# zju3dv/SMAP

Hardware: NVIDIA H100
Metric: end-to-end FPS @832x512 (backbone+association+lift) (higher is better)
Workload: dtype bf16x3 (split-bf16 operands, fp32 accumulate; fp32-faithful)

## Files before the change

### smap_b200/csrc/common.cuh

```cuda
#pragma once
#include <cuda_runtime.h>
#include <cuda_bf16.h>
#include <stdint.h>

#ifndef __CUDA_ARCH_FEAT_SM90_ALL
#if defined(__CUDA_ARCH__)
#error "smap_b200 kernels must be compiled with -gencode arch=compute_90a,code=sm_90a"
#endif
#endif

namespace smapb {

__device__ __forceinline__ uint32_t smem_u32(const void* p) {
    return (uint32_t)__cvta_generic_to_shared(p);
}

__device__ __forceinline__ void mbar_init(uint64_t* bar, uint32_t count) {
    asm volatile("mbarrier.init.shared::cta.b64 [%0], %1;" ::"r"(smem_u32(bar)), "r"(count) : "memory");
}
__device__ __forceinline__ void fence_mbar_init() {
    asm volatile("fence.mbarrier_init.release.cluster;" ::: "memory");
}
__device__ __forceinline__ void fence_proxy_async() {
    asm volatile("fence.proxy.async.shared::cta;" ::: "memory");
}
__device__ __forceinline__ void mbar_arrive_expect_tx(uint64_t* bar, uint32_t bytes) {
    asm volatile("mbarrier.arrive.expect_tx.shared::cta.b64 _, [%0], %1;" ::"r"(smem_u32(bar)), "r"(bytes)
                 : "memory");
}
__device__ __forceinline__ void mbar_arrive(uint64_t* bar) {
    asm volatile("mbarrier.arrive.shared::cta.b64 _, [%0];" ::"r"(smem_u32(bar)) : "memory");
}
__device__ __forceinline__ uint32_t mbar_try_wait(uint64_t* bar, uint32_t parity) {
    uint32_t ok;
    asm volatile(
        "{\n\t.reg .pred p;\n\t"
        "mbarrier.try_wait.parity.shared::cta.b64 p, [%1], %2;\n\t"
        "selp.u32 %0, 1, 0, p;\n\t}"
        : "=r"(ok)
        : "r"(smem_u32(bar)), "r"(parity)
        : "memory");
    return ok;
}
__device__ __forceinline__ void mbar_wait(uint64_t* bar, uint32_t parity) {
    if (mbar_try_wait(bar, parity)) return;
    const long long t0 = clock64();
    while (!mbar_try_wait(bar, parity)) {
        if (clock64() - t0 > 4000000000LL) {
            __trap();
        }
    }
}

__device__ __forceinline__ void bulk_g2s(void* dst_smem, const void* src_gmem, uint32_t bytes, uint64_t* bar) {
    asm volatile(
        "cp.async.bulk.shared::cluster.global.mbarrier::complete_tx::bytes [%0], [%1], %2, [%3];" ::"r"(
            smem_u32(dst_smem)),
        "l"(src_gmem), "r"(bytes), "r"(smem_u32(bar))
        : "memory");
}

__device__ __forceinline__ uint32_t lane_id() { return threadIdx.x & 31; }

__device__ __forceinline__ void pdl_wait() { asm volatile("griddepcontrol.wait;" ::: "memory"); }
__device__ __forceinline__ void pdl_trigger() { asm volatile("griddepcontrol.launch_dependents;" ::: "memory"); }

__device__ __forceinline__ void split_bf16(float v, __nv_bfloat16& hi, __nv_bfloat16& lo) {
    hi = __float2bfloat16_rn(v);
    lo = __float2bfloat16_rn(v - __bfloat162float(hi));
}
__device__ __forceinline__ uint32_t pack_bf16x2(__nv_bfloat16 a, __nv_bfloat16 b) {
    return (uint32_t)__bfloat16_as_ushort(a) | ((uint32_t)__bfloat16_as_ushort(b) << 16);
}
__device__ __forceinline__ float bf16lo_to_f(uint32_t packed) { return __uint_as_float(packed << 16); }
__device__ __forceinline__ float bf16hi_to_f(uint32_t packed) { return __uint_as_float(packed & 0xffff0000u); }

}
```

### smap_b200/csrc/conv_tc.cuh

```cuda
#pragma once
#include <cuda.h>
#include "common.cuh"

namespace smapb {

struct alignas(64) ConvParams {
    CUtensorMap tmA;
    CUtensorMap tmA2;
    CUtensorMap tmB;
    CUtensorMap tmO;
    CUtensorMap tmR[3];
    int Hout, Wout, Nimg;
    int tw_log2, th;
    int tiles_x, tiles_y;
    int Cout;
    int kh, kw, stride, pad_y, pad_x;
    int kchunks;
    int kchunks2, stride2;
    int n_tiles;
    int total_tiles;
    const float* bias;
    int has_res;
    int n_post;
    __nv_bfloat16* out;
    float* out_f32;
    long long plane_stride;
    int relu;
    int reverse;
    int up_mode, up_Hi, up_Wi, up_pw, up_ph;
    long long* dbg;
    long long* dbg_tl;
};

__device__ __forceinline__ void tma_load_5d(uint32_t dst, const CUtensorMap* map, uint64_t* bar, int c0, int c1,
                                            int c2, int c3, int c4) {
    asm volatile(
        "cp.async.bulk.tensor.5d.shared::cluster.global.tile.mbarrier::complete_tx::bytes [%0], [%1, {%3, %4, %5, %6, "
        "%7}], [%2];" ::"r"(dst),
        "l"(map), "r"(smem_u32(bar)), "r"(c0), "r"(c1), "r"(c2), "r"(c3), "r"(c4)
        : "memory");
}
__device__ __forceinline__ void tma_load_4d(uint32_t dst, const CUtensorMap* map, uint64_t* bar, int c0, int c1,
                                            int c2, int c3) {
    asm volatile(
        "cp.async.bulk.tensor.4d.shared::cluster.global.tile.mbarrier::complete_tx::bytes [%0], [%1, {%3, %4, %5, "
        "%6}], [%2];" ::"r"(dst),
        "l"(map), "r"(smem_u32(bar)), "r"(c0), "r"(c1), "r"(c2), "r"(c3)
        : "memory");
}
__device__ __forceinline__ void tma_prefetch_desc(const CUtensorMap* map) {
    asm volatile("prefetch.tensormap [%0];" ::"l"(map) : "memory");
}
__device__ __forceinline__ void tma_store_5d(const CUtensorMap* map, uint32_t src, int c0, int c1, int c2, int c3,
                                             int c4) {
    asm volatile("cp.async.bulk.tensor.5d.global.shared::cta.tile.bulk_group [%0, {%2, %3, %4, %5, %6}], [%1];" ::"l"(map),
                 "r"(src), "r"(c0), "r"(c1), "r"(c2), "r"(c3), "r"(c4)
                 : "memory");
}
__device__ __forceinline__ void bulk_commit() { asm volatile("cp.async.bulk.commit_group;" ::: "memory"); }
template <int N>
__device__ __forceinline__ void bulk_wait_read() {
    asm volatile("cp.async.bulk.wait_group.read %0;" ::"n"(N) : "memory");
}
__device__ __forceinline__ void bulk_wait_all() { asm volatile("cp.async.bulk.wait_group 0;" ::: "memory"); }
__device__ __forceinline__ void epi_bar_sync() { asm volatile("bar.sync 1, 256;" ::: "memory"); }
__device__ __forceinline__ uint32_t lds_u32(uint32_t addr) {
    uint32_t r;
    asm volatile("ld.shared.u32 %0, [%1];" : "=r"(r) : "r"(addr));
    return r;
}
__device__ __forceinline__ void sts_u32(uint32_t addr, uint32_t v) {
    asm volatile("st.shared.u32 [%0], %1;" ::"r"(addr), "r"(v) : "memory");
}
__device__ __forceinline__ uint32_t sw64_off(int r, int j) { return (uint32_t)(r * 64 + ((j ^ ((r >> 1) & 3)) << 4)); }

__device__ __forceinline__ float up_scale(int in, int out) { return out > 1 ? (float)(in - 1) / (float)(out - 1) : 0.f; }
__device__ __forceinline__ int up_src_index(int dst, int in, int out) { return (int)(up_scale(in, out) * (float)dst); }

__device__ __forceinline__ uint32_t cvt_bf16x2(float a, float b) {
    uint32_t w;
    asm("cvt.rn.bf16x2.f32 %0, %1, %2;" : "=r"(w) : "f"(b), "f"(a));
    return w;
}
__device__ __forceinline__ float2 planes_to_f2(uint32_t h, uint32_t l) {
    return make_float2(bf16lo_to_f(h) + bf16lo_to_f(l), bf16hi_to_f(h) + bf16hi_to_f(l));
}

__device__ __forceinline__ uint64_t wgmma_desc_sw128(uint32_t smem_addr) {
    uint64_t d = 0;
    d |= (uint64_t)((smem_addr >> 4) & 0x3FFF);
    d |= (uint64_t)1 << 16;
    d |= (uint64_t)(1024 >> 4) << 32;
    d |= (uint64_t)1 << 62;
    return d;
}
__device__ __forceinline__ void wgmma_fence() { asm volatile("wgmma.fence.sync.aligned;" ::: "memory"); }
__device__ __forceinline__ void wgmma_commit() { asm volatile("wgmma.commit_group.sync.aligned;" ::: "memory"); }
template <int N>
__device__ __forceinline__ void wgmma_wait() {
    asm volatile("wgmma.wait_group.sync.aligned %0;" ::"n"(N) : "memory");
}
__device__ __forceinline__ void wgmma_m64n128(float (&d)[64], uint64_t adesc, uint64_t bdesc, uint32_t accumulate) {
    asm volatile(
        "{\n\t.reg .pred p;\n\tsetp.ne.b32 p, %66, 0;\n\t"
        "wgmma.mma_async.sync.aligned.m64n128k16.f32.bf16.bf16 {%0, %1, %2, %3, %4, %5, %6, %7, %8, %9, %10, %11, %12, "
        "%13, %14, %15, %16, %17, %18, %19, %20, %21, %22, %23, %24, %25, %26, %27, %28, %29, %30, %31, %32, %33, %34, %35, "
        "%36, %37, %38, %39, %40, %41, %42, %43, %44, %45, %46, %47, %48, %49, %50, %51, %52, %53, %54, %55, %56, %57, %58, "
        "%59, %60, %61, %62, %63}, %64, %65, p, 1, 1, 0, 0;\n\t}"
        : "+f"(d[0]), "+f"(d[1]), "+f"(d[2]), "+f"(d[3]), "+f"(d[4]), "+f"(d[5]), "+f"(d[6]), "+f"(d[7]), "+f"(d[8]),
          "+f"(d[9]), "+f"(d[10]), "+f"(d[11]), "+f"(d[12]), "+f"(d[13]), "+f"(d[14]), "+f"(d[15]), "+f"(d[16]),
          "+f"(d[17]), "+f"(d[18]), "+f"(d[19]), "+f"(d[20]), "+f"(d[21]), "+f"(d[22]), "+f"(d[23]), "+f"(d[24]),
          "+f"(d[25]), "+f"(d[26]), "+f"(d[27]), "+f"(d[28]), "+f"(d[29]), "+f"(d[30]), "+f"(d[31]), "+f"(d[32]),
          "+f"(d[33]), "+f"(d[34]), "+f"(d[35]), "+f"(d[36]), "+f"(d[37]), "+f"(d[38]), "+f"(d[39]), "+f"(d[40]),
          "+f"(d[41]), "+f"(d[42]), "+f"(d[43]), "+f"(d[44]), "+f"(d[45]), "+f"(d[46]), "+f"(d[47]), "+f"(d[48]),
          "+f"(d[49]), "+f"(d[50]), "+f"(d[51]), "+f"(d[52]), "+f"(d[53]), "+f"(d[54]), "+f"(d[55]), "+f"(d[56]),
          "+f"(d[57]), "+f"(d[58]), "+f"(d[59]), "+f"(d[60]), "+f"(d[61]), "+f"(d[62]), "+f"(d[63])
        : "l"(adesc), "l"(bdesc), "r"(accumulate));
}
__device__ __forceinline__ void wgmma_m64n64(float (&d)[32], uint64_t adesc, uint64_t bdesc, uint32_t accumulate) {
    asm volatile(
        "{\n\t.reg .pred p;\n\tsetp.ne.b32 p, %34, 0;\n\t"
        "wgmma.mma_async.sync.aligned.m64n64k16.f32.bf16.bf16 {%0, %1, %2, %3, %4, %5, %6, %7, %8, %9, %10, %11, %12, "
        "%13, %14, %15, %16, %17, %18, %19, %20, %21, %22, %23, %24, %25, %26, %27, %28, %29, %30, %31}, %32, %33, p, 1, "
        "1, 0, 0;\n\t}"
        : "+f"(d[0]), "+f"(d[1]), "+f"(d[2]), "+f"(d[3]), "+f"(d[4]), "+f"(d[5]), "+f"(d[6]), "+f"(d[7]), "+f"(d[8]),
          "+f"(d[9]), "+f"(d[10]), "+f"(d[11]), "+f"(d[12]), "+f"(d[13]), "+f"(d[14]), "+f"(d[15]), "+f"(d[16]),
          "+f"(d[17]), "+f"(d[18]), "+f"(d[19]), "+f"(d[20]), "+f"(d[21]), "+f"(d[22]), "+f"(d[23]), "+f"(d[24]),
          "+f"(d[25]), "+f"(d[26]), "+f"(d[27]), "+f"(d[28]), "+f"(d[29]), "+f"(d[30]), "+f"(d[31])
        : "l"(adesc), "l"(bdesc), "r"(accumulate));
}
__device__ __forceinline__ void wgmma_m64n32(float (&d)[16], uint64_t adesc, uint64_t bdesc, uint32_t accumulate) {
    asm volatile(
        "{\n\t.reg .pred p;\n\tsetp.ne.b32 p, %18, 0;\n\t"
        "wgmma.mma_async.sync.aligned.m64n32k16.f32.bf16.bf16 {%0, %1, %2, %3, %4, %5, %6, %7, %8, %9, %10, %11, %12, "
        "%13, %14, %15}, %16, %17, p, 1, 1, 0, 0;\n\t}"
        : "+f"(d[0]), "+f"(d[1]), "+f"(d[2]), "+f"(d[3]), "+f"(d[4]), "+f"(d[5]), "+f"(d[6]), "+f"(d[7]), "+f"(d[8]),
          "+f"(d[9]), "+f"(d[10]), "+f"(d[11]), "+f"(d[12]), "+f"(d[13]), "+f"(d[14]), "+f"(d[15])
        : "l"(adesc), "l"(bdesc), "r"(accumulate));
}
template <int BLOCK_N>
__device__ __forceinline__ void wgmma_tile(float (&d)[BLOCK_N / 2], uint64_t adesc, uint64_t bdesc, uint32_t accumulate) {
    if constexpr (BLOCK_N == 128) wgmma_m64n128(d, adesc, bdesc, accumulate);
    else if constexpr (BLOCK_N == 64) wgmma_m64n64(d, adesc, bdesc, accumulate);
    else wgmma_m64n32(d, adesc, bdesc, accumulate);
}

__device__ __forceinline__ long long mbar_wait_timed(uint64_t* bar, uint32_t parity, bool timed) {
    if (!timed) {
        mbar_wait(bar, parity);
        return 0;
    }
    const long long t0 = clock64();
    mbar_wait(bar, parity);
    return clock64() - t0;
}

template <int BLOCK_N, int NTERMS, int RING>
struct ConvCfg {
    static constexpr int TA = (NTERMS == 3) ? 2 : 1;
    static constexpr int A_BYTES = 128 * 128;
    static constexpr int B_BYTES = BLOCK_N * 128;
    static constexpr int STAGE_BYTES = TA * (A_BYTES + B_BYTES);
    static constexpr int CHUNKS = BLOCK_N / 32;
    static constexpr int CHUNK_BYTES = 128 * 64;
    static constexpr int SLOT_BYTES = TA * CHUNK_BYTES;
    static constexpr int OUT_BUFS = 2;
    static constexpr int RES_BUFS = RING ? 2 : 0;
    static constexpr int RES_DIV = RING ? RES_BUFS : 1;
    static constexpr int EPI_BYTES = (OUT_BUFS + RES_BUFS) * SLOT_BYTES;
    static constexpr int SMEM_LIMIT = 227 * 1024;
    static constexpr int STAGES_RAW = (SMEM_LIMIT - 2048 - EPI_BYTES) / STAGE_BYTES;
    static constexpr int STAGES = STAGES_RAW > 8 ? 8 : STAGES_RAW;
    static constexpr int SMEM_BYTES = STAGES * STAGE_BYTES + EPI_BYTES + 2048;
    static_assert(STAGES >= 2, "need at least a double buffer");
    static_assert(BLOCK_N == 32 || BLOCK_N == 64 || BLOCK_N == 128, "BLOCK_N");
};

template <int BLOCK_N, int NTERMS, int RING>
__global__ void __launch_bounds__(384, 1) conv_tc_kernel(const __grid_constant__ ConvParams p) {
    using Cfg = ConvCfg<BLOCK_N, NTERMS, RING>;
    constexpr int STAGES = Cfg::STAGES;
    constexpr bool UP = (RING == 2);
    extern __shared__ unsigned char smem_raw[];
    uint64_t* full_bar = reinterpret_cast<uint64_t*>(smem_raw);
    uint64_t* empty_bar = full_bar + STAGES;
    uint64_t* rfull_bar = empty_bar + STAGES;
    uint64_t* rempty_bar = rfull_bar + Cfg::RES_BUFS;
    const uint32_t ring = (smem_u32(smem_raw) + 1024u + 1023u) & ~1023u;
    const uint32_t out_stage = ring + STAGES * Cfg::STAGE_BYTES;
    const uint32_t res_stage = out_stage + Cfg::OUT_BUFS * Cfg::SLOT_BYTES;

    const int warp = threadIdx.x >> 5;
    const int lane = threadIdx.x & 31;
    const bool tl = p.dbg_tl != nullptr && blockIdx.x == 0;
    if (tl && threadIdx.x == 0) p.dbg_tl[0] = clock64();
    const int n_extra = RING ? p.has_res + p.n_post : 0;
    const bool tma_out = p.out != nullptr;

    if (warp == 0 && lane == 0) {
        tma_prefetch_desc(&p.tmA);
        tma_prefetch_desc(&p.tmB);
        if (p.kchunks2) tma_prefetch_desc(&p.tmA2);
        if (tma_out) tma_prefetch_desc(&p.tmO);
        for (int e = 0; e < n_extra; e++) tma_prefetch_desc(&p.tmR[e]);
    }
    if (warp == 1 && lane == 0) {
        for (int s = 0; s < STAGES; s++) {
            mbar_init(&full_bar[s], 1);
            mbar_init(&empty_bar[s], 8);
        }
        for (int s = 0; s < Cfg::RES_BUFS; s++) {
            mbar_init(&rfull_bar[s], 1);
            mbar_init(&rempty_bar[s], 256);
        }
        fence_mbar_init();
    }
    __syncthreads();

    const int num_kb1 = p.kh * p.kw * p.kchunks;
    const int num_kb = num_kb1 + p.kchunks2;
    const int tiles_per_img = p.tiles_x * p.tiles_y;
    const int tw = 1 << p.tw_log2;

    if (tl && threadIdx.x == 0) p.dbg_tl[1] = clock64();
    pdl_wait();
    pdl_trigger();

    if (warp == 0) {
        if (lane == 0) {
            int stage = 0;
            uint32_t phase = 0;
            long long w_empty = 0;
            for (int tile = blockIdx.x; tile < p.total_tiles; tile += gridDim.x) {
                const int te = p.reverse ? p.total_tiles - 1 - tile : tile;
                const int nt = te % p.n_tiles, mt = te / p.n_tiles;
                const int img = mt / tiles_per_img, r = mt - img * tiles_per_img;
                const int ty = r / p.tiles_x, tx = r - ty * p.tiles_x;
                const int x_in0 = (tx << p.tw_log2) * p.stride - p.pad_x;
                const int y_in0 = ty * p.th * p.stride - p.pad_y;
                for (int kb = 0; kb < num_kb; kb++) {
                    w_empty += mbar_wait_timed(&empty_bar[stage], phase ^ 1u, p.dbg != nullptr);
                    const uint32_t sbase = ring + stage * Cfg::STAGE_BYTES;
                    mbar_arrive_expect_tx(&full_bar[stage], Cfg::STAGE_BYTES);
                    const int brow = nt * BLOCK_N;
                    int kcol, tapc, ax, ay;
                    const CUtensorMap* amap;
                    if (kb < num_kb1) {
                        const int ts = kb / p.kchunks, kc = kb - ts * p.kchunks;
                        const int kx = ts / p.kh, ky = ts - kx * p.kh;
                        amap = &p.tmA, kcol = kc * 64, tapc = ky * p.kw + kx, ax = x_in0 + kx, ay = y_in0 + ky;
                    } else {
                        const int kc2 = kb - num_kb1;
                        amap = &p.tmA2, kcol = kc2 * 64, tapc = 0;
                        ax = (tx << p.tw_log2) * p.stride2, ay = ty * p.th * p.stride2;
                    }
                    const int wcol = (kb < num_kb1) ? kcol : (p.kchunks * 64 + kcol);
#pragma unroll
                    for (int t = 0; t < Cfg::TA; t++) {
                        const uint32_t da = sbase + t * Cfg::A_BYTES, db = sbase + Cfg::TA * Cfg::A_BYTES + t * Cfg::B_BYTES;
                        tma_load_5d(da, amap, &full_bar[stage], kcol, ax, ay, img, t);
                        tma_load_4d(db, &p.tmB, &full_bar[stage], wcol, brow, tapc, t);
                    }
                    if (++stage == STAGES) {
                        stage = 0;
                        phase ^= 1u;
                    }
                }
            }
            if (p.dbg) atomicAdd((unsigned long long*)&p.dbg[0], (unsigned long long)w_empty);
        }
    } else if (warp == 1) {
        if (lane == 0 && n_extra > 0) {
            int cnt = 0;
            for (int tile = blockIdx.x; tile < p.total_tiles; tile += gridDim.x) {
                const int te = p.reverse ? p.total_tiles - 1 - tile : tile;
                const int nt = te % p.n_tiles, mt = te / p.n_tiles;
                const int img = mt / tiles_per_img, r = mt - img * tiles_per_img;
                const int ty = r / p.tiles_x, tx = r - ty * p.tiles_x;
                for (int c = 0; c < Cfg::CHUNKS; c++) {
                    for (int e = 0; e < n_extra; e++) {
                        const int m = cnt++;
                        const int slot = m % Cfg::RES_DIV;
                        mbar_wait(&rempty_bar[slot], ((uint32_t)(m / Cfg::RES_DIV) & 1u) ^ 1u);
                        int cx = tx << p.tw_log2, cy = ty * p.th;
                        uint32_t bytes = Cfg::SLOT_BYTES;
                        if (UP && e == 0) {
                            cx = up_src_index(cx, p.up_Wi, p.Wout);
                            cy = up_src_index(cy, p.up_Hi, p.Hout);
                            bytes = (uint32_t)(p.up_pw * p.up_ph * 64 * Cfg::TA);
                        }
                        mbar_arrive_expect_tx(&rfull_bar[slot], bytes);
#pragma unroll
                        for (int t = 0; t < Cfg::TA; t++)
                            tma_load_5d(res_stage + slot * Cfg::SLOT_BYTES + t * Cfg::CHUNK_BYTES, &p.tmR[e],
                                        &rfull_bar[slot], nt * BLOCK_N + c * 32, cx, cy, img, t);
                    }
                }
            }
        }
    } else if (warp >= 4) {
        const int ct = threadIdx.x - 128;
        const int wg = ct >> 7;
        const int q4 = lane & 3;
        const int row0 = wg * 64 + ((ct >> 5) & 3) * 16 + (lane >> 2);
        const bool leader = (ct == 0);
        int stage = 0;
        uint32_t phase = 0;
        int rcnt = 0, ocnt = 0;
        long long w_full = 0, w_stage = 0, w_ring = 0;
        const long long t_begin = (p.dbg && leader) ? clock64() : 0;
        float acc[BLOCK_N / 2];
        for (int tile = blockIdx.x; tile < p.total_tiles; tile += gridDim.x) {
            const int te = p.reverse ? p.total_tiles - 1 - tile : tile;
            const int nt = te % p.n_tiles, mt = te / p.n_tiles;
            const int img = mt / tiles_per_img, r = mt - img * tiles_per_img;
            const int ty = r / p.tiles_x, tx = r - ty * p.tiles_x;
            const int n0 = nt * BLOCK_N;

            int prev_stage = -1;
            for (int kb = 0; kb < num_kb; kb++) {
                w_full += mbar_wait_timed(&full_bar[stage], phase, p.dbg != nullptr && leader);
                if (tl && leader && tile == (int)blockIdx.x && kb == 0) p.dbg_tl[2] = clock64();
                const uint32_t sbase = ring + stage * Cfg::STAGE_BYTES;
                const uint64_t a0 = wgmma_desc_sw128(sbase + (uint32_t)(wg * 64 * 128));
                const uint64_t b0 = wgmma_desc_sw128(sbase + Cfg::TA * Cfg::A_BYTES);
                constexpr uint64_t A_STEP = (uint64_t)(Cfg::A_BYTES >> 4), B_STEP = (uint64_t)(Cfg::B_BYTES >> 4);
                wgmma_fence();
#pragma unroll
                for (int k = 0; k < 4; k++) {
                    const uint64_t ka = a0 + (uint64_t)(k * 2), kbd = b0 + (uint64_t)(k * 2);
                    wgmma_tile<BLOCK_N>(acc, ka, kbd, (kb | k) != 0);
                    if (NTERMS == 3) {
                        wgmma_tile<BLOCK_N>(acc, ka + A_STEP, kbd, 1u);
                        wgmma_tile<BLOCK_N>(acc, ka, kbd + B_STEP, 1u);
                    }
                }
                wgmma_commit();
                wgmma_wait<1>();
                if (prev_stage >= 0 && lane == 0) mbar_arrive(&empty_bar[prev_stage]);
                prev_stage = stage;
                if (++stage == STAGES) {
                    stage = 0;
                    phase ^= 1u;
                }
            }
            wgmma_wait<0>();
            if (lane == 0) mbar_arrive(&empty_bar[prev_stage]);
            if (tl && leader && tile + (int)gridDim.x >= p.total_tiles) p.dbg_tl[3] = clock64();

            int py[2], px[2];
            bool valid[2];
            long long pix[2];
#pragma unroll
            for (int i = 0; i < 2; i++) {
                const int row = row0 + 8 * i;
                py[i] = ty * p.th + (row >> p.tw_log2);
                px[i] = (tx << p.tw_log2) + (row & (tw - 1));
                valid[i] = (py[i] < p.Hout) && (px[i] < p.Wout) && (img < p.Nimg);
                pix[i] = ((long long)img * p.Hout + py[i]) * p.Wout + px[i];
            }
            auto ring_wait = [&]() -> uint32_t {
                const int m = rcnt++;
                const int rslot = m % Cfg::RES_DIV;
                w_ring += mbar_wait_timed(&rfull_bar[rslot], (uint32_t)(m / Cfg::RES_DIV) & 1u, p.dbg != nullptr && leader);
                return (uint32_t)rslot;
            };
            auto ring_release = [&](uint32_t rslot) {
                fence_proxy_async();
                mbar_arrive(&rempty_bar[rslot]);
            };
            auto ring_add = [&](float(&vv)[2][8]) {
                const uint32_t rslot = ring_wait();
                const uint32_t rb = res_stage + rslot * Cfg::SLOT_BYTES;
                float2 rv[2][4];
#pragma unroll
                for (int i = 0; i < 2; i++)
#pragma unroll
                    for (int jj = 0; jj < 4; jj++) {
                        const uint32_t o = sw64_off(row0 + 8 * i, jj) + 4 * q4;
                        rv[i][jj] = planes_to_f2(lds_u32(rb + o), NTERMS == 3 ? lds_u32(rb + Cfg::CHUNK_BYTES + o) : 0u);
                    }
                ring_release(rslot);
#pragma unroll
                for (int i = 0; i < 2; i++)
#pragma unroll
                    for (int jj = 0; jj < 4; jj++) {
                        vv[i][2 * jj] += rv[i][jj].x;
                        vv[i][2 * jj + 1] += rv[i][jj].y;
                    }
            };
#pragma unroll
            for (int c = 0; c < Cfg::CHUNKS; c++) {
                const int c0 = c * 32;
                float v[2][8];
#pragma unroll
                for (int jj = 0; jj < 4; jj++) {
                    const float2 bia = __ldg(reinterpret_cast<const float2*>(p.bias + n0 + c0 + 8 * jj + 2 * q4));
                    const int j = 4 * c + jj;
                    v[0][2 * jj] = acc[4 * j + 0] + bia.x;
                    v[0][2 * jj + 1] = acc[4 * j + 1] + bia.y;
                    v[1][2 * jj] = acc[4 * j + 2] + bia.x;
                    v[1][2 * jj + 1] = acc[4 * j + 3] + bia.y;
                }
                if (RING == 1 && p.has_res) ring_add(v);
                if (UP) {
                    const uint32_t rslot = ring_wait();
                    const uint32_t rb = res_stage + rslot * Cfg::SLOT_BYTES;
                    const int oy0 = up_src_index(ty * p.th, p.up_Hi, p.Hout), ox0 = up_src_index(tx << p.tw_log2, p.up_Wi, p.Wout);
                    float upv[2][8];
#pragma unroll
                    for (int i = 0; i < 2; i++) {
                        const int pyc = min(py[i], p.Hout - 1), pxc = min(px[i], p.Wout - 1);
                        const float sy = up_scale(p.up_Hi, p.Hout) * (float)pyc, sx = up_scale(p.up_Wi, p.Wout) * (float)pxc;
                        const int y0i = (int)sy, x0i = (int)sx;
                        const int y1i = y0i + (y0i < p.up_Hi - 1 ? 1 : 0), x1i = x0i + (x0i < p.up_Wi - 1 ? 1 : 0);
                        const float hy1 = sy - (float)y0i, hy0 = 1.f - hy1, wx1 = sx - (float)x0i, wx0 = 1.f - wx1;
                        const int rr[4] = {(y0i - oy0) * p.up_pw + (x0i - ox0), (y0i - oy0) * p.up_pw + (x1i - ox0),
                                           (y1i - oy0) * p.up_pw + (x0i - ox0), (y1i - oy0) * p.up_pw + (x1i - ox0)};
#pragma unroll
                        for (int jj = 0; jj < 4; jj++) {
                            float2 q[4];
#pragma unroll
                            for (int k = 0; k < 4; k++) {
                                const uint32_t o = sw64_off(rr[k], jj) + 4 * q4;
                                q[k] = planes_to_f2(lds_u32(rb + o), NTERMS == 3 ? lds_u32(rb + Cfg::CHUNK_BYTES + o) : 0u);
                            }
                            upv[i][2 * jj] = hy0 * (wx0 * q[0].x + wx1 * q[1].x) + hy1 * (wx0 * q[2].x + wx1 * q[3].x);
                            upv[i][2 * jj + 1] = hy0 * (wx0 * q[0].y + wx1 * q[1].y) + hy1 * (wx0 * q[2].y + wx1 * q[3].y);
                        }
                    }
                    ring_release(rslot);
#pragma unroll
                    for (int i = 0; i < 2; i++)
#pragma unroll
                        for (int e = 0; e < 8; e++) v[i][e] += upv[i][e];
                }
                if (p.relu) {
#pragma unroll
                    for (int i = 0; i < 2; i++)
#pragma unroll
                        for (int e = 0; e < 8; e++) v[i][e] = fmaxf(v[i][e], 0.f);
                }
                for (int e = 0; RING == 1 && e < p.n_post; e++) ring_add(v);
                if (tma_out) {
                    const uint32_t ob = out_stage + (uint32_t)(ocnt & 1) * Cfg::SLOT_BYTES;
                    ocnt++;
                    if (leader) {
                        const long long t0 = p.dbg ? clock64() : 0;
                        bulk_wait_read<1>();
                        if (p.dbg) w_stage += clock64() - t0;
                    }
                    epi_bar_sync();
#pragma unroll
                    for (int i = 0; i < 2; i++)
#pragma unroll
                        for (int jj = 0; jj < 4; jj++) {
                            const float a = v[i][2 * jj], b = v[i][2 * jj + 1];
                            const uint32_t hw = cvt_bf16x2(a, b);
                            const uint32_t o = sw64_off(row0 + 8 * i, jj) + 4 * q4;
                            sts_u32(ob + o, hw);
                            if (NTERMS == 3)
                                sts_u32(ob + Cfg::CHUNK_BYTES + o, cvt_bf16x2(a - bf16lo_to_f(hw), b - bf16hi_to_f(hw)));
                        }
                    fence_proxy_async();
                    epi_bar_sync();
                    if (leader) {
#pragma unroll
                        for (int t = 0; t < Cfg::TA; t++)
                            tma_store_5d(&p.tmO, ob + t * Cfg::CHUNK_BYTES, n0 + c0, tx << p.tw_log2, ty * p.th, img, t);
                        bulk_commit();
                    }
                } else {
#pragma unroll
                    for (int i = 0; i < 2; i++) {
                        if (!valid[i]) continue;
#pragma unroll
                        for (int jj = 0; jj < 4; jj++)
                            *reinterpret_cast<float2*>(p.out_f32 + pix[i] * p.Cout + n0 + c0 + 8 * jj + 2 * q4) =
                                make_float2(v[i][2 * jj], v[i][2 * jj + 1]);
                    }
                }
            }
        }
        if (leader && tma_out) bulk_wait_all();
        if (tl && leader) p.dbg_tl[13] = clock64();
        if (p.dbg && leader) {
            atomicAdd((unsigned long long*)&p.dbg[1], (unsigned long long)w_full);
            atomicAdd((unsigned long long*)&p.dbg[4], (unsigned long long)w_stage);
            atomicAdd((unsigned long long*)&p.dbg[9], (unsigned long long)w_ring);
            atomicAdd((unsigned long long*)&p.dbg[7], (unsigned long long)(clock64() - t_begin));
            atomicAdd((unsigned long long*)&p.dbg[8], 1ull);
        }
    }
    __syncthreads();
    if (tl && threadIdx.x == 0) p.dbg_tl[15] = clock64();
}

}
```

### smap_b200/csrc/engine.cu

```cuda
#include <cuda.h>
#include <cuda_runtime.h>
#include <dlfcn.h>
#include <math.h>
#include <nvtx3/nvToolsExt.h>
#include <stdio.h>
#include <stdlib.h>
#include <string.h>

#include <algorithm>
#include <map>
#include <memory>
#include <mutex>
#include <string>
#include <vector>

#include "../../include/smap_b200.h"
#include "../../include/smap_b200_debug.h"
#include "assoc.h"
#include "conv_tc.cuh"
#include "elementwise.h"
#include "preprocess.h"
#include "refine.h"

using namespace smapb;
// ... 2071 lines not shown
        CK(cudaMemcpy(&sums[n], d, 8, cudaMemcpyDeviceToHost));
        if (desc) snprintf(desc + (size_t)n * desc_stride, desc_stride, "%s", buf);
        n++;
    }
    cudaFree(d);
    return n;
}

int64_t smapb_launch_count(const smapb_handle* h) { return h ? h->launches : 0; }

int smapb_profile_begin(smapb_handle* h) {
    if (!h) return -1;
    h->profiling = true;
    h->prof_used = 0;
    if (getenv("SMAPB_ROLES_PLAN")) {
        cudaSetDevice(h->device);
        if (!h->roles_dev) CK(cudaMalloc((void**)&h->roles_dev, ROLES_CAP * 16 * sizeof(long long)));
        CK(cudaMemset(h->roles_dev, 0, ROLES_CAP * 16 * sizeof(long long)));
        h->roles_used = 0;
        h->roles_desc.clear();
    }
    return 0;
}

int smapb_profile_end(smapb_handle* h, double* ms_by_kind, int* launches_by_kind, const char* csv_path) {
    if (!h) return -1;
    cudaSetDevice(h->device);
    h->profiling = false;
    CK(cudaDeviceSynchronize());
    for (int k = 0; k < 6; k++) {
        if (ms_by_kind) ms_by_kind[k] = 0;
        if (launches_by_kind) launches_by_kind[k] = 0;
    }
    FILE* f = csv_path ? fopen(csv_path, "w") : nullptr;
    if (f) fprintf(f, "idx,kind,ms,gflop,tflops,desc\n");
    for (size_t i = 1; i < h->prof_used; i++) {
        const int k = h->prof_kind[i];
        if (k < 0) continue;
        float ms = 0;
        cudaEventElapsedTime(&ms, h->prof_events[i - 1], h->prof_events[i]);
        if (ms_by_kind) ms_by_kind[k] += ms;
        if (launches_by_kind) launches_by_kind[k]++;
        if (f)
            fprintf(f, "%zu,%d,%.5f,%.4f,%.2f,%s\n", i, k, ms, h->prof_flops[i] * 1e-9,
                    ms > 0 ? h->prof_flops[i] / (ms * 1e-3) * 1e-12 : 0.0, h->prof_desc[i].c_str());
    }
    if (f) fclose(f);
    h->prof_used = 0;
    if (h->roles_dev && h->roles_used && getenv("SMAPB_ROLES_PLAN")) {
        std::vector<long long> d(h->roles_used * 16);
        CK(cudaMemcpy(d.data(), h->roles_dev, d.size() * sizeof(long long), cudaMemcpyDeviceToHost));
        FILE* g = fopen(getenv("SMAPB_ROLES_PLAN"), "w");
        if (g) {
            fprintf(g, "idx,name,desc,issuers,total,producer_wait_empty,mma_wait_full,mma_wait_tempty,g0_wait_tfull,g0_wait_stage,"
                       "g0_wait_ring,g1_wait_tfull,g1_wait_stage,g1_wait_ring\n");
            for (size_t i = 0; i < h->roles_used && i < h->roles_desc.size(); i++) {
                const long long* r = &d[i * 16];
                const double n = r[8] > 0 ? (double)r[8] : 1.0;
                const double cg = (strstr(h->roles_desc[i].c_str(), " cg2 ") || strstr(h->roles_desc[i].c_str(), " cg3 ")) ? 2.0 : 1.0;
                fprintf(g, "%zu,%s,%.0f,%.0f,%.0f,%.0f,%.0f,%.0f,%.0f,%.0f,%.0f,%.0f,%.0f\n", i, h->roles_desc[i].c_str(), n,
                        r[7] / n, r[0] / n / cg, r[1] / n, r[2] / n, r[3] / n / cg, r[4] / n / cg, r[9] / n / cg, r[5] / n / cg,
                        r[6] / n / cg, r[10] / n / cg);
            }
            fclose(g);
        }
        h->roles_used = 0;
    }
    return 0;
}

int smapb_plan_info(const smapb_handle* hc, int B, int* n_conv, double* conv_flops) {
    smapb_handle* h = const_cast<smapb_handle*>(hc);
    if (!h) return -1;
    if (!h->finalized) return fail(h, -2, "weights not finalized");
    cudaSetDevice(h->device);
    Plan* plan = nullptr;
    int rc = build_plan(h, B, &plan);
    if (rc) return rc;
    if (n_conv) *n_conv = plan->n_conv;
    if (conv_flops) *conv_flops = plan->conv_flops;
    return 0;
}

__global__ void split_to_f32_kernel(const __nv_bfloat16* __restrict__ in, long long plane, int terms, float* __restrict__ out,
                                    long long n) {
    const long long i = (long long)blockIdx.x * blockDim.x + threadIdx.x;
    if (i >= n) return;
    float v = __bfloat162float(in[i]);
    if (terms == 2) v += __bfloat162float(in[plane + i]);
    out[i] = v;
}

int smapb_conv_test(smapb_handle* h, const float* x, const float* w, const float* bias, const float* res,
                    const float* post1, const float* post2, int B, int H, int W, int Cin, int Cout, int k, int stride,
                    int relu, int precision, float* y, float* ms_out, void* stream) {
    if (!h) return -1;
    cudaSetDevice(h->device);
    cudaStream_t st = (cudaStream_t)stream;
    const int save_terms = h->nterms, save_planes = h->planes;
    h->nterms = precision == SMAPB_PREC_BF16 ? 1 : 3;
    h->planes = precision == SMAPB_PREC_BF16 ? 1 : 2;
    int rc = 0;
    ConvLayer L;
    L.name = "conv_test";
    L.Cin = Cin, L.Cout = Cout, L.Cout_pad = pad32(Cout), L.k = k, L.stride = stride, L.pad = k / 2, L.relu = relu;
    std::vector<float> wh((size_t)Cout * Cin * k * k), bh(Cout);
    std::vector<void*> tmp;
    auto cleanup = [&]() {
        for (void* p : tmp) cudaFree(p);
        cudaFree(L.w_dev);
        cudaFree(L.bias_dev);
        h->nterms = save_terms;
        h->planes = save_planes;
    };
#define CKT(call)                                                                         \
// ... 17 lines not shown
    out.N = B, out.H = Ho, out.W = Wo, out.C = L.Cout_pad;
    r = out;
    p1 = out;
    p2 = out;
    void* p = nullptr;
    CKT(cudaMalloc(&p, (size_t)in.plane() * 2 * h->planes));
    tmp.push_back(p);
    in.ptr = (__nv_bfloat16*)p;
    CKT(cudaMalloc(&p, (size_t)out.plane() * 2 * h->planes));
    tmp.push_back(p);
    out.ptr = (__nv_bfloat16*)p;
    CKT(cudaMemset(p, 0, (size_t)out.plane() * 2 * h->planes));
    CKT(launch_f32_to_split(x, in.ptr, in.plane(), in.plane(), h->planes, st));
    const float* extra_src[3] = {res, post1, post2};
    Act* extra_act[3] = {&r, &p1, &p2};
    for (int e = 0; e < 3; e++) {
        if (!extra_src[e]) continue;
        if (L.Cout_pad != Cout) {
            cleanup();
            return fail(h, -1, "conv_test: residual/post operands require Cout % 32 == 0");
        }
        CKT(cudaMalloc(&p, (size_t)out.plane() * 2 * h->planes));
        tmp.push_back(p);
        extra_act[e]->ptr = (__nv_bfloat16*)p;
        CKT(launch_f32_to_split(extra_src[e], extra_act[e]->ptr, out.plane(), out.plane(), h->planes, st));
    }
    ConvParams cp;
    int bn = 0;
    rc = setup_conv(h, L, in, res ? &r : nullptr, post1 ? &p1 : nullptr, post2 ? &p2 : nullptr, &out, nullptr, relu,
                    &cp, &bn, nullptr);
    if (rc) {
        cleanup();
        return rc;
    }
    cudaEvent_t e0, e1;
    cudaEventCreate(&e0);
    cudaEventCreate(&e1);
    long long* dbg_dev = nullptr;
    if (getenv("SMAPB_ROLES")) {
        CKT(cudaMalloc((void**)&dbg_dev, 16 * sizeof(long long)));
        tmp.push_back(dbg_dev);
        CKT(cudaMemset(dbg_dev, 0, 16 * sizeof(long long)));
        cp.dbg = dbg_dev;
    }
    long long* tl_dev = nullptr;
    if (getenv("SMAPB_TIMELINE")) {
        CKT(cudaMalloc((void**)&tl_dev, 16 * sizeof(long long)));
        tmp.push_back(tl_dev);
    }
    CKT(launch_conv(cp, bn, h->nterms, h->sm_count, st, false));
    if (dbg_dev) {
        long long d[16];
        CKT(cudaMemcpy(d, dbg_dev, sizeof d, cudaMemcpyDeviceToHost));
        const double n = d[8] > 0 ? (double)d[8] : 1.0;
        fprintf(stderr,
                "[roles] bn%d units%d kb%d | mean cycles per CTA: total %.0f | producer wait-empty %.0f | consumer wait-full %.0f "
                "wait-stage %.0f wait-ring %.0f\n",
                bn, cp.total_tiles, cp.kh * cp.kw * cp.kchunks + cp.kchunks2, d[7] / n, d[0] / n, d[1] / n, d[4] / n, d[9] / n);
        cp.dbg = nullptr;
    }
    if (tl_dev) {
        CKT(cudaMemset(tl_dev, 0, 16 * sizeof(long long)));
        cp.dbg_tl = tl_dev;
        CKT(launch_conv(cp, bn, h->nterms, h->sm_count, st, false));
        cp.dbg_tl = nullptr;
        long long t[16];
        CKT(cudaMemcpy(t, tl_dev, sizeof t, cudaMemcpyDeviceToHost));
        fprintf(stderr, "[timeline] bn%d units%d kb%d | set-up %lld | first operands %lld | last main loop end %lld | epilogue done "
                "%lld | exit %lld\n", bn, cp.total_tiles, cp.kh * cp.kw * cp.kchunks + cp.kchunks2, t[1] - t[0], t[2] - t[0],
                t[3] - t[0], t[13] - t[0], t[15] - t[0]);
    }
    const int reps = ms_out ? 5 : 0;
    cudaEventRecord(e0, st);
    for (int i = 0; i < reps; i++) CKT(launch_conv(cp, bn, h->nterms, h->sm_count, st, false));
    cudaEventRecord(e1, st);
    h->launches += 1 + reps;
    float* ytmp = nullptr;
    CKT(cudaMalloc((void**)&ytmp, (size_t)out.plane() * 4));
    tmp.push_back(ytmp);
    split_to_f32_kernel<<<(unsigned)((out.plane() + 255) / 256), 256, 0, st>>>(out.ptr, out.plane(), h->planes, ytmp,
                                                                               out.plane());
    CKT(cudaGetLastError());
    CKT(cudaMemcpy2DAsync(y, (size_t)Cout * 4, ytmp, (size_t)L.Cout_pad * 4, (size_t)Cout * 4, (size_t)B * Ho * Wo,
                          cudaMemcpyDeviceToDevice, st));
    CKT(cudaStreamSynchronize(st));
    if (ms_out) {
        float ms = 0;
        cudaEventElapsedTime(&ms, e0, e1);
        *ms_out = ms / reps;
    }
    cudaEventDestroy(e0);
    cudaEventDestroy(e1);
    cleanup();
    return 0;
#undef CKT
}

#pragma GCC visibility pop
}
```

Before: 449.7.

## Ping-pong two consumer warpgroups over alternating full 128-row conv tiles

Each of the two consumer warpgroups now computes an entire 128-row tile on its own, and the two alternate tiles, using named-barrier turn passing for both the main loop and the residual ring. One warpgroup's epilogue can then overlap with the other's wgmma main loop. Register budgets are rebalanced with setmaxnreg so producers drop to 40 registers and consumers rise to 232, which leaves room for the doubled accumulators. The change also gives each warpgroup its own output staging buffers when that costs no pipeline stage, adjusts the mbarrier arrival counts, and reworks the debug counters. The risks are register pressure from the two accumulator sets and tighter ordering constraints between the warpgroups.

```diff
diff --git a/smap_b200/csrc/common.cuh b/smap_b200/csrc/common.cuh
--- a/smap_b200/csrc/common.cuh
+++ b/smap_b200/csrc/common.cuh
@@ -42,12 +42,13 @@
         : "memory");
     return ok;
 }
+static __device__ __noinline__ void mbar_timeout() { __trap(); }
 __device__ __forceinline__ void mbar_wait(uint64_t* bar, uint32_t parity) {
     if (mbar_try_wait(bar, parity)) return;
     const long long t0 = clock64();
     while (!mbar_try_wait(bar, parity)) {
         if (clock64() - t0 > 4000000000LL) {
-            __trap();
+            mbar_timeout();
         }
     }
 }
diff --git a/smap_b200/csrc/conv_tc.cuh b/smap_b200/csrc/conv_tc.cuh
--- a/smap_b200/csrc/conv_tc.cuh
+++ b/smap_b200/csrc/conv_tc.cuh
@@ -63,7 +63,33 @@
     asm volatile("cp.async.bulk.wait_group.read %0;" ::"n"(N) : "memory");
 }
 __device__ __forceinline__ void bulk_wait_all() { asm volatile("cp.async.bulk.wait_group 0;" ::: "memory"); }
-__device__ __forceinline__ void epi_bar_sync() { asm volatile("bar.sync 1, 256;" ::: "memory"); }
+enum { TURN_MAIN = 3, TURN_RING = 5 };
+__device__ __forceinline__ void epi_bar_sync(int wg) { asm volatile("bar.sync %0, 128;" ::"r"(1 + wg) : "memory"); }
+__device__ __forceinline__ void turn_wait(int turn, int wg) { asm volatile("bar.sync %0, 256;" ::"r"(turn + wg) : "memory"); }
+__device__ __forceinline__ void turn_pass(int turn, int wg) { asm volatile("bar.arrive %0, 256;" ::"r"(turn + wg) : "memory"); }
+template <int R>
+__device__ __forceinline__ void setmaxnreg_dec() {
+    asm volatile("setmaxnreg.dec.sync.aligned.u32 %0;" ::"n"(R));
+}
+template <int R>
+__device__ __forceinline__ void setmaxnreg_inc() {
+    asm volatile("setmaxnreg.inc.sync.aligned.u32 %0;" ::"n"(R));
+}
+struct ConvDbg {
+    enum {
+        PRODUCER_WAIT_EMPTY = 0,
+        TOTAL = 1,
+        CTAS = 2,
+        CONS = 3,
+        WAIT_FULL = 0,
+        WAIT_ORDER = 1,
+        EPILOGUE = 2,
+        WAIT_RING = 3,
+        WAIT_STAGE = 4,
+        CONS_N = 5,
+        COUNT = CONS + 2 * CONS_N
+    };
+};
 __device__ __forceinline__ uint32_t lds_u32(uint32_t addr) {
     uint32_t r;
     asm volatile("ld.shared.u32 %0, [%1];" : "=r"(r) : "r"(addr));
@@ -164,13 +190,18 @@
     static constexpr int CHUNKS = BLOCK_N / 32;
     static constexpr int CHUNK_BYTES = 128 * 64;
     static constexpr int SLOT_BYTES = TA * CHUNK_BYTES;
-    static constexpr int OUT_BUFS = 2;
     static constexpr int RES_BUFS = RING ? 2 : 0;
     static constexpr int RES_DIV = RING ? RES_BUFS : 1;
+    static constexpr int SMEM_LIMIT = 227 * 1024;
+    static constexpr int stages_with(int out_bufs) {
+        return (SMEM_LIMIT - 2048 - (out_bufs + RES_BUFS) * SLOT_BYTES) / STAGE_BYTES > 8
+                   ? 8
+                   : (SMEM_LIMIT - 2048 - (out_bufs + RES_BUFS) * SLOT_BYTES) / STAGE_BYTES;
+    }
+    static constexpr int OUT_PER_WG = stages_with(4) == stages_with(2) ? 2 : 1;
+    static constexpr int OUT_BUFS = 2 * OUT_PER_WG;
     static constexpr int EPI_BYTES = (OUT_BUFS + RES_BUFS) * SLOT_BYTES;
-    static constexpr int SMEM_LIMIT = 227 * 1024;
-    static constexpr int STAGES_RAW = (SMEM_LIMIT - 2048 - EPI_BYTES) / STAGE_BYTES;
-    static constexpr int STAGES = STAGES_RAW > 8 ? 8 : STAGES_RAW;
+    static constexpr int STAGES = stages_with(OUT_BUFS);
     static constexpr int SMEM_BYTES = STAGES * STAGE_BYTES + EPI_BYTES + 2048;
     static_assert(STAGES >= 2, "need at least a double buffer");
     static_assert(BLOCK_N == 32 || BLOCK_N == 64 || BLOCK_N == 128, "BLOCK_N");
@@ -207,11 +238,11 @@
     if (warp == 1 && lane == 0) {
         for (int s = 0; s < STAGES; s++) {
             mbar_init(&full_bar[s], 1);
-            mbar_init(&empty_bar[s], 8);
+            mbar_init(&empty_bar[s], 4);
         }
         for (int s = 0; s < Cfg::RES_BUFS; s++) {
             mbar_init(&rfull_bar[s], 1);
-            mbar_init(&rempty_bar[s], 256);
+            mbar_init(&rempty_bar[s], 128);
         }
         fence_mbar_init();
     }
@@ -225,9 +256,11 @@
     if (tl && threadIdx.x == 0) p.dbg_tl[1] = clock64();
     pdl_wait();
     pdl_trigger();
-
-    if (warp == 0) {
-        if (lane == 0) {
+    const long long t_begin = p.dbg ? clock64() : 0;
+
+    if (warp < 4) {
+        setmaxnreg_dec<40>();
+        if (warp == 0 && lane == 0) {
             int stage = 0;
             uint32_t phase = 0;
             long long w_empty = 0;
@@ -267,10 +300,8 @@
                     }
                 }
             }
-            if (p.dbg) atomicAdd((unsigned long long*)&p.dbg[0], (unsigned long long)w_empty);
-        }
-    } else if (warp == 1) {
-        if (lane == 0 && n_extra > 0) {
+            if (p.dbg) atomicAdd((unsigned long long*)&p.dbg[ConvDbg::PRODUCER_WAIT_EMPTY], (unsigned long long)w_empty);
+        } else if (warp == 1 && lane == 0 && n_extra > 0) {
             int cnt = 0;
             for (int tile = blockIdx.x; tile < p.total_tiles; tile += gridDim.x) {
                 const int te = p.reverse ? p.total_tiles - 1 - tile : tile;
@@ -298,41 +329,57 @@
                 }
             }
         }
-    } else if (warp >= 4) {
-        const int ct = threadIdx.x - 128;
-        const int wg = ct >> 7;
+    } else {
+        setmaxnreg_inc<232>();
+        const int wg = (warp >> 2) - 1;
         const int q4 = lane & 3;
-        const int row0 = wg * 64 + ((ct >> 5) & 3) * 16 + (lane >> 2);
-        const bool leader = (ct == 0);
-        int stage = 0;
-        uint32_t phase = 0;
-        int rcnt = 0, ocnt = 0;
-        long long w_full = 0, w_stage = 0, w_ring = 0;
-        const long long t_begin = (p.dbg && leader) ? clock64() : 0;
-        float acc[BLOCK_N / 2];
-        for (int tile = blockIdx.x; tile < p.total_tiles; tile += gridDim.x) {
+        const int rw = (warp & 3) * 16 + (lane >> 2);
+        const bool leader = (threadIdx.x & 127) == 0;
+        const bool timed = p.dbg != nullptr && leader;
+        const uint32_t ob0 = out_stage + (uint32_t)(wg * Cfg::OUT_PER_WG) * Cfg::SLOT_BYTES;
+        const int n_cta = (p.total_tiles - (int)blockIdx.x + (int)gridDim.x - 1) / (int)gridDim.x;
+        long long* const dc = p.dbg ? p.dbg + ConvDbg::CONS + ConvDbg::CONS_N * wg : nullptr;
+        auto tally = [&](int k, long long cycles) {
+            if (timed) atomicAdd((unsigned long long*)&dc[k], (unsigned long long)cycles);
+        };
+        float acc[2][BLOCK_N / 2];
+        for (int j = wg; j < n_cta; j += 2) {
+            const int tile = blockIdx.x + j * gridDim.x;
             const int te = p.reverse ? p.total_tiles - 1 - tile : tile;
             const int nt = te % p.n_tiles, mt = te / p.n_tiles;
             const int img = mt / tiles_per_img, r = mt - img * tiles_per_img;
             const int ty = r / p.tiles_x, tx = r - ty * p.tiles_x;
             const int n0 = nt * BLOCK_N;
 
+            const uint32_t it0 = (uint32_t)j * (uint32_t)num_kb;
+            int stage = (int)(it0 % STAGES);
+            uint32_t phase = (it0 / STAGES) & 1u;
+            if (j > 0) {
+                const long long t0 = timed ? clock64() : 0;
+                turn_wait(TURN_MAIN, wg);
+                tally(ConvDbg::WAIT_ORDER, timed ? clock64() - t0 : 0);
+            }
             int prev_stage = -1;
+            uint32_t w_full = 0;
             for (int kb = 0; kb < num_kb; kb++) {
-                w_full += mbar_wait_timed(&full_bar[stage], phase, p.dbg != nullptr && leader);
-                if (tl && leader && tile == (int)blockIdx.x && kb == 0) p.dbg_tl[2] = clock64();
+                w_full += (uint32_t)mbar_wait_timed(&full_bar[stage], phase, timed);
+                if (tl && leader && j == 0 && kb == 0) p.dbg_tl[2] = clock64();
                 const uint32_t sbase = ring + stage * Cfg::STAGE_BYTES;
-                const uint64_t a0 = wgmma_desc_sw128(sbase + (uint32_t)(wg * 64 * 128));
+                const uint64_t a0 = wgmma_desc_sw128(sbase);
                 const uint64_t b0 = wgmma_desc_sw128(sbase + Cfg::TA * Cfg::A_BYTES);
                 constexpr uint64_t A_STEP = (uint64_t)(Cfg::A_BYTES >> 4), B_STEP = (uint64_t)(Cfg::B_BYTES >> 4);
+                constexpr uint64_t A_HALF = (uint64_t)((64 * 128) >> 4);
                 wgmma_fence();
 #pragma unroll
                 for (int k = 0; k < 4; k++) {
-                    const uint64_t ka = a0 + (uint64_t)(k * 2), kbd = b0 + (uint64_t)(k * 2);
-                    wgmma_tile<BLOCK_N>(acc, ka, kbd, (kb | k) != 0);
-                    if (NTERMS == 3) {
-                        wgmma_tile<BLOCK_N>(acc, ka + A_STEP, kbd, 1u);
-                        wgmma_tile<BLOCK_N>(acc, ka, kbd + B_STEP, 1u);
+#pragma unroll
+                    for (int h = 0; h < 2; h++) {
+                        const uint64_t ka = a0 + (uint64_t)(k * 2) + h * A_HALF, kbd = b0 + (uint64_t)(k * 2);
+                        wgmma_tile<BLOCK_N>(acc[h], ka, kbd, (kb | k) != 0);
+                        if (NTERMS == 3) {
+                            wgmma_tile<BLOCK_N>(acc[h], ka + A_STEP, kbd, 1u);
+                            wgmma_tile<BLOCK_N>(acc[h], ka, kbd + B_STEP, 1u);
+                        }
                     }
                 }
                 wgmma_commit();
@@ -344,73 +391,76 @@
                     phase ^= 1u;
                 }
             }
+            if (j + 1 < n_cta) turn_pass(TURN_MAIN, wg ^ 1);
+            tally(ConvDbg::WAIT_FULL, w_full);
             wgmma_wait<0>();
             if (lane == 0) mbar_arrive(&empty_bar[prev_stage]);
-            if (tl && leader && tile + (int)gridDim.x >= p.total_tiles) p.dbg_tl[3] = clock64();
-
-            int py[2], px[2];
-            bool valid[2];
-            long long pix[2];
-#pragma unroll
-            for (int i = 0; i < 2; i++) {
-                const int row = row0 + 8 * i;
-                py[i] = ty * p.th + (row >> p.tw_log2);
-                px[i] = (tx << p.tw_log2) + (row & (tw - 1));
-                valid[i] = (py[i] < p.Hout) && (px[i] < p.Wout) && (img < p.Nimg);
-                pix[i] = ((long long)img * p.Hout + py[i]) * p.Wout + px[i];
-            }
+            if (tl && leader && j == n_cta - 1) p.dbg_tl[3] = clock64();
+
+            const long long t_epi0 = timed ? clock64() : 0;
+            int py[4], px[4];
+            bool valid[4];
+            long long pix[4];
+#pragma unroll
+            for (int q = 0; q < 4; q++) {
+                const int row = 64 * (q >> 1) + rw + 8 * (q & 1);
+                py[q] = ty * p.th + (row >> p.tw_log2);
+                px[q] = (tx << p.tw_log2) + (row & (tw - 1));
+                valid[q] = (py[q] < p.Hout) && (px[q] < p.Wout) && (img < p.Nimg);
+                pix[q] = ((long long)img * p.Hout + py[q]) * p.Wout + px[q];
+            }
+            auto row_of = [&](int q) { return 64 * (q >> 1) + rw + 8 * (q & 1); };
+            const bool ring_turns = RING != 0 && n_extra > 0;
+            if (ring_turns && j > 0) turn_wait(TURN_RING, wg);
+            int rcnt = j * Cfg::CHUNKS * n_extra;
             auto ring_wait = [&]() -> uint32_t {
                 const int m = rcnt++;
                 const int rslot = m % Cfg::RES_DIV;
-                w_ring += mbar_wait_timed(&rfull_bar[rslot], (uint32_t)(m / Cfg::RES_DIV) & 1u, p.dbg != nullptr && leader);
+                tally(ConvDbg::WAIT_RING, mbar_wait_timed(&rfull_bar[rslot], (uint32_t)(m / Cfg::RES_DIV) & 1u, timed));
                 return (uint32_t)rslot;
             };
             auto ring_release = [&](uint32_t rslot) {
                 fence_proxy_async();
                 mbar_arrive(&rempty_bar[rslot]);
             };
-            auto ring_add = [&](float(&vv)[2][8]) {
+            auto ring_add = [&](float(&vv)[4][8]) {
                 const uint32_t rslot = ring_wait();
                 const uint32_t rb = res_stage + rslot * Cfg::SLOT_BYTES;
-                float2 rv[2][4];
-#pragma unroll
-                for (int i = 0; i < 2; i++)
+#pragma unroll
+                for (int q = 0; q < 4; q++)
 #pragma unroll
                     for (int jj = 0; jj < 4; jj++) {
-                        const uint32_t o = sw64_off(row0 + 8 * i, jj) + 4 * q4;
-                        rv[i][jj] = planes_to_f2(lds_u32(rb + o), NTERMS == 3 ? lds_u32(rb + Cfg::CHUNK_BYTES + o) : 0u);
+                        const uint32_t o = sw64_off(row_of(q), jj) + 4 * q4;
+                        const float2 rv = planes_to_f2(lds_u32(rb + o), NTERMS == 3 ? lds_u32(rb + Cfg::CHUNK_BYTES + o) : 0u);
+                        vv[q][2 * jj] += rv.x;
+                        vv[q][2 * jj + 1] += rv.y;
                     }
                 ring_release(rslot);
-#pragma unroll
-                for (int i = 0; i < 2; i++)
-#pragma unroll
-                    for (int jj = 0; jj < 4; jj++) {
-                        vv[i][2 * jj] += rv[i][jj].x;
-                        vv[i][2 * jj + 1] += rv[i][jj].y;
-                    }
             };
 #pragma unroll
             for (int c = 0; c < Cfg::CHUNKS; c++) {
                 const int c0 = c * 32;
-                float v[2][8];
+                float v[4][8];
 #pragma unroll
                 for (int jj = 0; jj < 4; jj++) {
                     const float2 bia = __ldg(reinterpret_cast<const float2*>(p.bias + n0 + c0 + 8 * jj + 2 * q4));
-                    const int j = 4 * c + jj;
-                    v[0][2 * jj] = acc[4 * j + 0] + bia.x;
-                    v[0][2 * jj + 1] = acc[4 * j + 1] + bia.y;
-                    v[1][2 * jj] = acc[4 * j + 2] + bia.x;
-                    v[1][2 * jj + 1] = acc[4 * j + 3] + bia.y;
+                    const int f = 4 * (4 * c + jj);
+#pragma unroll
+                    for (int h = 0; h < 2; h++) {
+                        v[2 * h][2 * jj] = acc[h][f + 0] + bia.x;
+                        v[2 * h][2 * jj + 1] = acc[h][f + 1] + bia.y;
+                        v[2 * h + 1][2 * jj] = acc[h][f + 2] + bia.x;
+                        v[2 * h + 1][2 * jj + 1] = acc[h][f + 3] + bia.y;
+                    }
                 }
                 if (RING == 1 && p.has_res) ring_add(v);
                 if (UP) {
                     const uint32_t rslot = ring_wait();
                     const uint32_t rb = res_stage + rslot * Cfg::SLOT_BYTES;
                     const int oy0 = up_src_index(ty * p.th, p.up_Hi, p.Hout), ox0 = up_src_index(tx << p.tw_log2, p.up_Wi, p.Wout);
-                    float upv[2][8];
-#pragma unroll
-                    for (int i = 0; i < 2; i++) {
-                        const int pyc = min(py[i], p.Hout - 1), pxc = min(px[i], p.Wout - 1);
+#pragma unroll
+                    for (int q = 0; q < 4; q++) {
+                        const int pyc = min(py[q], p.Hout - 1), pxc = min(px[q], p.Wout - 1);
                         const float sy = up_scale(p.up_Hi, p.Hout) * (float)pyc, sx = up_scale(p.up_Wi, p.Wout) * (float)pxc;
                         const int y0i = (int)sy, x0i = (int)sx;
                         const int y1i = y0i + (y0i < p.up_Hi - 1 ? 1 : 0), x1i = x0i + (x0i < p.up_Wi - 1 ? 1 : 0);
@@ -419,51 +469,46 @@
                                            (y1i - oy0) * p.up_pw + (x0i - ox0), (y1i - oy0) * p.up_pw + (x1i - ox0)};
 #pragma unroll
                         for (int jj = 0; jj < 4; jj++) {
-                            float2 q[4];
+                            float2 s[4];
 #pragma unroll
                             for (int k = 0; k < 4; k++) {
                                 const uint32_t o = sw64_off(rr[k], jj) + 4 * q4;
-                                q[k] = planes_to_f2(lds_u32(rb + o), NTERMS == 3 ? lds_u32(rb + Cfg::CHUNK_BYTES + o) : 0u);
+                                s[k] = planes_to_f2(lds_u32(rb + o), NTERMS == 3 ? lds_u32(rb + Cfg::CHUNK_BYTES + o) : 0u);
                             }
-                            upv[i][2 * jj] = hy0 * (wx0 * q[0].x + wx1 * q[1].x) + hy1 * (wx0 * q[2].x + wx1 * q[3].x);
-                            upv[i][2 * jj + 1] = hy0 * (wx0 * q[0].y + wx1 * q[1].y) + hy1 * (wx0 * q[2].y + wx1 * q[3].y);
+                            v[q][2 * jj] += hy0 * (wx0 * s[0].x + wx1 * s[1].x) + hy1 * (wx0 * s[2].x + wx1 * s[3].x);
+                            v[q][2 * jj + 1] += hy0 * (wx0 * s[0].y + wx1 * s[1].y) + hy1 * (wx0 * s[2].y + wx1 * s[3].y);
                         }
                     }
                     ring_release(rslot);
-#pragma unroll
-                    for (int i = 0; i < 2; i++)
-#pragma unroll
-                        for (int e = 0; e < 8; e++) v[i][e] += upv[i][e];
                 }
                 if (p.relu) {
 #pragma unroll
-                    for (int i = 0; i < 2; i++)
-#pragma unroll
-                        for (int e = 0; e < 8; e++) v[i][e] = fmaxf(v[i][e], 0.f);
+                    for (int q = 0; q < 4; q++)
+#pragma unroll
+                        for (int e = 0; e < 8; e++) v[q][e] = fmaxf(v[q][e], 0.f);
                 }
                 for (int e = 0; RING == 1 && e < p.n_post; e++) ring_add(v);
                 if (tma_out) {
-                    const uint32_t ob = out_stage + (uint32_t)(ocnt & 1) * Cfg::SLOT_BYTES;
-                    ocnt++;
+                    const uint32_t ob = ob0 + (uint32_t)((((j >> 1) * Cfg::CHUNKS + c) % Cfg::OUT_PER_WG) * Cfg::SLOT_BYTES);
                     if (leader) {
-                        const long long t0 = p.dbg ? clock64() : 0;
-                        bulk_wait_read<1>();
-                        if (p.dbg) w_stage += clock64() - t0;
-                    }
-                    epi_bar_sync();
-#pragma unroll
-                    for (int i = 0; i < 2; i++)
+                        const long long t0 = timed ? clock64() : 0;
+                        bulk_wait_read<Cfg::OUT_PER_WG - 1>();
+                        tally(ConvDbg::WAIT_STAGE, timed ? clock64() - t0 : 0);
+                    }
+                    epi_bar_sync(wg);
+#pragma unroll
+                    for (int q = 0; q < 4; q++)
 #pragma unroll
                         for (int jj = 0; jj < 4; jj++) {
-                            const float a = v[i][2 * jj], b = v[i][2 * jj + 1];
+                            const float a = v[q][2 * jj], b = v[q][2 * jj + 1];
                             const uint32_t hw = cvt_bf16x2(a, b);
-                            const uint32_t o = sw64_off(row0 + 8 * i, jj) + 4 * q4;
+                            const uint32_t o = sw64_off(row_of(q), jj) + 4 * q4;
                             sts_u32(ob + o, hw);
                             if (NTERMS == 3)
                                 sts_u32(ob + Cfg::CHUNK_BYTES + o, cvt_bf16x2(a - bf16lo_to_f(hw), b - bf16hi_to_f(hw)));
                         }
                     fence_proxy_async();
-                    epi_bar_sync();
+                    epi_bar_sync(wg);
                     if (leader) {
 #pragma unroll
                         for (int t = 0; t < Cfg::TA; t++)
@@ -472,28 +517,27 @@
                     }
                 } else {
 #pragma unroll
-                    for (int i = 0; i < 2; i++) {
-                        if (!valid[i]) continue;
+                    for (int q = 0; q < 4; q++) {
+                        if (!valid[q]) continue;
 #pragma unroll
                         for (int jj = 0; jj < 4; jj++)
-                            *reinterpret_cast<float2*>(p.out_f32 + pix[i] * p.Cout + n0 + c0 + 8 * jj + 2 * q4) =
-                                make_float2(v[i][2 * jj], v[i][2 * jj + 1]);
-                    }
-                }
-            }
+                            *reinterpret_cast<float2*>(p.out_f32 + pix[q] * p.Cout + n0 + c0 + 8 * jj + 2 * q4) =
+                                make_float2(v[q][2 * jj], v[q][2 * jj + 1]);
+                    }
+                }
+            }
+            if (ring_turns && j + 1 < n_cta) turn_pass(TURN_RING, wg ^ 1);
+            tally(ConvDbg::EPILOGUE, timed ? clock64() - t_epi0 : 0);
         }
         if (leader && tma_out) bulk_wait_all();
-        if (tl && leader) p.dbg_tl[13] = clock64();
-        if (p.dbg && leader) {
-            atomicAdd((unsigned long long*)&p.dbg[1], (unsigned long long)w_full);
-            atomicAdd((unsigned long long*)&p.dbg[4], (unsigned long long)w_stage);
-            atomicAdd((unsigned long long*)&p.dbg[9], (unsigned long long)w_ring);
-            atomicAdd((unsigned long long*)&p.dbg[7], (unsigned long long)(clock64() - t_begin));
-            atomicAdd((unsigned long long*)&p.dbg[8], 1ull);
+        if (leader && wg == ((n_cta - 1) & 1)) {
+            if (p.dbg) {
+                atomicAdd((unsigned long long*)&p.dbg[ConvDbg::TOTAL], (unsigned long long)(clock64() - t_begin));
+                atomicAdd((unsigned long long*)&p.dbg[ConvDbg::CTAS], 1ull);
+            }
+            if (tl) p.dbg_tl[13] = p.dbg_tl[15] = clock64();
         }
     }
-    __syncthreads();
-    if (tl && threadIdx.x == 0) p.dbg_tl[15] = clock64();
-}
-
-}
+}
+
+}
diff --git a/smap_b200/csrc/engine.cu b/smap_b200/csrc/engine.cu
--- a/smap_b200/csrc/engine.cu
+++ b/smap_b200/csrc/engine.cu
@@ -2147,15 +2147,15 @@
         CK(cudaMemcpy(d.data(), h->roles_dev, d.size() * sizeof(long long), cudaMemcpyDeviceToHost));
         FILE* g = fopen(getenv("SMAPB_ROLES_PLAN"), "w");
         if (g) {
-            fprintf(g, "idx,name,desc,issuers,total,producer_wait_empty,mma_wait_full,mma_wait_tempty,g0_wait_tfull,g0_wait_stage,"
-                       "g0_wait_ring,g1_wait_tfull,g1_wait_stage,g1_wait_ring\n");
+            fprintf(g, "idx,name,desc,ctas,total,producer_wait_empty,g0_wait_full,g0_wait_order,g0_epilogue,g0_wait_ring,"
+                       "g0_wait_stage,g1_wait_full,g1_wait_order,g1_epilogue,g1_wait_ring,g1_wait_stage\n");
             for (size_t i = 0; i < h->roles_used && i < h->roles_desc.size(); i++) {
                 const long long* r = &d[i * 16];
-                const double n = r[8] > 0 ? (double)r[8] : 1.0;
-                const double cg = (strstr(h->roles_desc[i].c_str(), " cg2 ") || strstr(h->roles_desc[i].c_str(), " cg3 ")) ? 2.0 : 1.0;
-                fprintf(g, "%zu,%s,%.0f,%.0f,%.0f,%.0f,%.0f,%.0f,%.0f,%.0f,%.0f,%.0f,%.0f\n", i, h->roles_desc[i].c_str(), n,
-                        r[7] / n, r[0] / n / cg, r[1] / n, r[2] / n, r[3] / n / cg, r[4] / n / cg, r[9] / n / cg, r[5] / n / cg,
-                        r[6] / n / cg, r[10] / n / cg);
+                const double n = r[ConvDbg::CTAS] > 0 ? (double)r[ConvDbg::CTAS] : 1.0;
+                fprintf(g, "%zu,%s,%.0f,%.0f,%.0f", i, h->roles_desc[i].c_str(), n, r[ConvDbg::TOTAL] / n,
+                        r[ConvDbg::PRODUCER_WAIT_EMPTY] / n);
+                for (int c = ConvDbg::CONS; c < ConvDbg::COUNT; c++) fprintf(g, ",%.0f", r[c] / n);
+                fprintf(g, "\n");
             }
             fclose(g);
         }
@@ -2279,11 +2279,17 @@
     if (dbg_dev) {
         long long d[16];
         CKT(cudaMemcpy(d, dbg_dev, sizeof d, cudaMemcpyDeviceToHost));
-        const double n = d[8] > 0 ? (double)d[8] : 1.0;
-        fprintf(stderr,
-                "[roles] bn%d units%d kb%d | mean cycles per CTA: total %.0f | producer wait-empty %.0f | consumer wait-full %.0f "
-                "wait-stage %.0f wait-ring %.0f\n",
-                bn, cp.total_tiles, cp.kh * cp.kw * cp.kchunks + cp.kchunks2, d[7] / n, d[0] / n, d[1] / n, d[4] / n, d[9] / n);
+        const double n = d[ConvDbg::CTAS] > 0 ? (double)d[ConvDbg::CTAS] : 1.0;
+        fprintf(stderr, "[roles] bn%d units%d kb%d | mean cycles per CTA: total %.0f | producer wait-empty %.0f", bn,
+                cp.total_tiles, cp.kh * cp.kw * cp.kchunks + cp.kchunks2, d[ConvDbg::TOTAL] / n,
+                d[ConvDbg::PRODUCER_WAIT_EMPTY] / n);
+        for (int g = 0; g < 2; g++) {
+            const long long* c = d + ConvDbg::CONS + ConvDbg::CONS_N * g;
+            fprintf(stderr, " | g%d wait-full %.0f wait-order %.0f epilogue %.0f wait-ring %.0f wait-stage %.0f", g,
+                    c[ConvDbg::WAIT_FULL] / n, c[ConvDbg::WAIT_ORDER] / n, c[ConvDbg::EPILOGUE] / n, c[ConvDbg::WAIT_RING] / n,
+                    c[ConvDbg::WAIT_STAGE] / n);
+        }
+        fprintf(stderr, "\n");
         cp.dbg = nullptr;
     }
     if (tl_dev) {
```

After: 473.8 (median of 6 runs). 5.4% higher.
